# UCL/gp_emulator

Hardware: AMD Instinct MI355X
Metric: test-points/sec for predict(mean+var+grad), N_train=250 D=11 (higher is better)
Workload: dtype f64

## Files before the change

### gp_emulator_amd/csrc/gp_predict_kernel.hpp

```cpp
#pragma once
#include <hip/hip_runtime.h>
#include <stdint.h>
#include <type_traits>
#include <utility>

namespace gpk {

#ifndef GP_WAVES
#define GP_WAVES 8
#endif
#ifndef GP_WAVES_F32
#define GP_WAVES_F32 12
#endif
#ifndef GP_CHUNK
#define GP_CHUNK 64
#endif
#ifndef GP_CHUNK_F32
#define GP_CHUNK_F32 192
#endif
#ifndef GP_ABLATE
#define GP_ABLATE 0
#endif
#ifndef GP_AHEAD
#define GP_AHEAD 4
#endif
#ifndef GP_AHEAD_F32
#define GP_AHEAD_F32 8
#endif
#ifndef GP_RING_PIN
#define GP_RING_PIN 1
#endif
#ifndef GP_MU_DOUBLE
#define GP_MU_DOUBLE 1
#endif
#ifndef GP_ESTRIN
#define GP_ESTRIN 0
#endif
#ifndef GP_EXP_FUSED
#define GP_EXP_FUSED 1
#endif
#ifndef GP_DOTSPLIT
#define GP_DOTSPLIT 1
#endif
#ifndef GP_GROUP_F64
#define GP_GROUP_F64 1
#endif
#ifndef GP_STAMPS
#define GP_STAMPS 0
#endif
constexpr int kTile = 16;
template <typename T, bool kVar = true> struct Geo {
  static constexpr int kWaves = sizeof(T) == 8 ? GP_WAVES : GP_WAVES_F32;
  static constexpr int kThreads = kWaves * 64;
#ifndef GP_WG_PER_CU_SMALL
#define GP_WG_PER_CU_SMALL 0
#endif
  static constexpr int kWGPerCU = kWaves >= 8 ? 1 : (GP_WG_PER_CU_SMALL > 0 ? GP_WG_PER_CU_SMALL : 8 / kWaves);
  static constexpr int kWavesPerSimd = kWaves >= 8 ? kWaves / 4 : kWGPerCU * kWaves / 4;
  static constexpr int kRowsPerWG = kWaves * kTile;
  static constexpr int kChunk = sizeof(T) == 8 ? GP_CHUNK : GP_CHUNK_F32;
};
#ifndef GP_MG_WAVES
#define GP_MG_WAVES 12
#endif
#ifndef GP_MG_WAVES_F32
#define GP_MG_WAVES_F32 16
#endif
#ifndef GP_MG_WG_PER_CU
#define GP_MG_WG_PER_CU 1
#endif
template <typename T> struct Geo<T, false> {
  static constexpr int kWaves = sizeof(T) == 8 ? GP_MG_WAVES : GP_MG_WAVES_F32;
  static constexpr int kThreads = kWaves * 64;
  static constexpr int kWGPerCU = GP_MG_WG_PER_CU;
  static constexpr int kWavesPerSimd = kWGPerCU * kWaves / 4;
  static constexpr int kRowsPerWG = kWaves * kTile;
  static constexpr int kChunk = 1;
};

typedef double f64x4 __attribute__((ext_vector_type(4)));
typedef float f32x4 __attribute__((ext_vector_type(4)));

template <typename F, int... Is>
__device__ __forceinline__ void static_for_impl(F&& f, std::integer_sequence<int, Is...>) {
  (f(std::integral_constant<int, Is>{}), ...);
}
template <int N, typename F>
__device__ __forceinline__ void static_for(F&& f) {
  static_for_impl(f, std::make_integer_sequence<int, N>{});
}

template <typename T> struct Real;
template <> struct Real<double> {
  typedef f64x4 acc_t;
  static constexpr bool kExpand = true;
  static constexpr int kGroup = GP_GROUP_F64;
  __host__ __device__ static constexpr int own_sub(int r, int g) { return 4 * r + g; }
  __device__ static inline acc_t mfma(double a, double b, acc_t c) {
    return __builtin_amdgcn_mfma_f64_16x16x4f64(a, b, c, 0, 0, 0);
  }
  static constexpr double kRoundMagic = 6755399441055744.0;
  __host__ __device__ static inline double exp_(double x) {
#if GP_EXP_FUSED
    const double s = fma(x, 1.4426950408889634, kRoundMagic);
    const double n = s - kRoundMagic;
    const int ni = (int)(unsigned)__builtin_bit_cast(unsigned long long, s);
#else
    x = __builtin_fmax(x, -1000.0);
    const double n = __builtin_rint(x * 1.4426950408889634);
    const int ni = (int)n;
#endif
    double r = fma(n, -6.93147180559945286e-01, x);
    r = fma(n, -2.31904681384629956e-17, r);
#if GP_ESTRIN
    const double r2 = r * r;
    const double p01 = fma(1.00000000000000666e+00, r, 1.0);
    const double p23 = fma(1.66666666665544028e-01, r, 5.00000000000000555e-01);
    const double p45 = fma(8.33333338566834801e-03, r, 4.16666666665732183e-02);
    const double p67 = fma(1.98411702695461072e-04, r, 1.38888889324666632e-03);
    const double p89 = fma(2.76401812311866076e-06, r, 2.48015043709117912e-05);
    const double r4 = r2 * r2;
    const double q0 = fma(r2, p23, p01);
    const double q1 = fma(r2, p67, p45);
    const double q2 = fma(r2, 2.76263485910095559e-07, p89);
    const double r8 = r4 * r4;
    const double s0 = fma(r4, q1, q0);
    const double p = fma(r8, q2, s0);
#else
    double p = 2.76263485910095559e-07;
    p = fma(p, r, 2.76401812311866076e-06);
    p = fma(p, r, 2.48015043709117912e-05);
    p = fma(p, r, 1.98411702695461072e-04);
    p = fma(p, r, 1.38888889324666632e-03);
    p = fma(p, r, 8.33333338566834801e-03);
    p = fma(p, r, 4.16666666665732183e-02);
    p = fma(p, r, 1.66666666665544028e-01);
    p = fma(p, r, 5.00000000000000555e-01);
    p = fma(p, r, 1.00000000000000666e+00);
    p = fma(p, r, 1.0);
#endif
    return ldexp(p, ni);
  }
  __host__ __device__ static inline double exp_clamped(double x) { return exp_(__builtin_fmax(x, -1000.0)); }
  template <int GP>
  __device__ static inline void exp_n(double (&x)[GP]) {
    double n[GP], r[GP], p[GP];
    int ni[GP];
#pragma unroll
    for (int u = 0; u < GP; ++u) x[u] = __builtin_fmax(x[u], -1000.0);
#if GP_EXP_FUSED
#pragma unroll
    for (int u = 0; u < GP; ++u) r[u] = fma(x[u], 1.4426950408889634, kRoundMagic);
#pragma unroll
    for (int u = 0; u < GP; ++u) {
      n[u] = r[u] - kRoundMagic;
      ni[u] = (int)(unsigned)__builtin_bit_cast(unsigned long long, r[u]);
    }
#else
#pragma unroll
    for (int u = 0; u < GP; ++u) {
      n[u] = __builtin_rint(x[u] * 1.4426950408889634);
      ni[u] = (int)n[u];
    }
#endif
#pragma unroll
    for (int u = 0; u < GP; ++u) r[u] = fma(n[u], -6.93147180559945286e-01, x[u]);
#pragma unroll
    for (int u = 0; u < GP; ++u) r[u] = fma(n[u], -2.31904681384629956e-17, r[u]);
#pragma unroll
    for (int u = 0; u < GP; ++u) p[u] = 2.76263485910095559e-07;
    constexpr double c[10] = {2.76401812311866076e-06, 2.48015043709117912e-05, 1.98411702695461072e-04,
                              1.38888889324666632e-03, 8.33333338566834801e-03, 4.16666666665732183e-02,
                              1.66666666665544028e-01, 5.00000000000000555e-01, 1.00000000000000666e+00, 1.0};
#pragma unroll
    for (int j = 0; j < 10; ++j) {
#pragma unroll
      for (int u = 0; u < GP; ++u) p[u] = fma(p[u], r[u], c[j]);
    }
#pragma unroll
    for (int u = 0; u < GP; ++u) x[u] = ldexp(p[u], ni[u]);
  }
  static constexpr double kMaxHalfNorm2 = 67108864.0;
  static constexpr double kFarG = 134217728.0;
};
template <> struct Real<float> {
  typedef f32x4 acc_t;
  static constexpr bool kExpand = false;
#ifndef GP_GROUP_F32
#define GP_GROUP_F32 2
#endif
  static constexpr int kGroup = GP_GROUP_F32;
  __host__ __device__ static constexpr int own_sub(int r, int g) { return 4 * g + r; }
  __device__ static inline acc_t mfma(float a, float b, acc_t c) {
    return __builtin_amdgcn_mfma_f32_16x16x4f32(a, b, c, 0, 0, 0);
  }
  __device__ static inline float exp_(float x) { return __expf(x); }
  __device__ static inline float exp_clamped(float x) { return __expf(x); }
  template <int GP>
  __device__ static inline void exp_n(float (&x)[GP]) {
#pragma unroll
    for (int u = 0; u < GP; ++u) x[u] = __expf(x[u]);
  }
};

template <typename T>
__host__ __device__ constexpr int own_index(int I, int s, int g) {
  return 16 * I + Real<T>::own_sub(s, g);
}

template <typename T>
__host__ __device__ constexpr int point_slot(int n) {
  return 16 * (n / 16) + Real<T>::own_sub((n % 16) / 4, n % 4);
}
template <typename T>
__host__ __device__ constexpr int slot_point(int slot) {
  for (int q = 0; q < 16; ++q)
    if (Real<T>::own_sub(q / 4, q % 4) == slot % 16) return 16 * (slot / 16) + q;
  return -1;
}

struct FragId { int I, J, s; };
__host__ __device__ constexpr int frag_count(int NB) { return NB * (NB + 1) / 2 * 4; }
__host__ __device__ constexpr int frag_col_offset(int J, int NB) { return J * NB - J * (J - 1) / 2; }
__host__ __device__ constexpr FragId frag_at(int n, int NB) {
  const int pair = n >> 2;
  int J = 0;
  while (J + 1 < NB && frag_col_offset(J + 1, NB) <= pair) ++J;
  return FragId{J + pair - frag_col_offset(J, NB), J, n & 3};
}
__host__ __device__ constexpr int frag_index(int I, int J, int s, int NB) {
  return (frag_col_offset(J, NB) + (I - J)) * 4 + s;
}
__host__ __device__ constexpr int frag_count_padded(int NB, int chunk) {
  return (frag_count(NB) + chunk - 1) / chunk * chunk;
}

__host__ __device__ constexpr int row_stride(int D) { return (D + 2 + 3) & ~3; }
#ifndef GP_XA_PAD
#define GP_XA_PAD 1
#endif
template <typename T> __host__ __device__ constexpr int xa_lds_stride(int D) {
  return (GP_XA_PAD && sizeof(T) == 4 && row_stride(D) % 16 == 0) ? row_stride(D) + 4 : row_stride(D);
}

#ifndef GP_FRAG_BUFS
#define GP_FRAG_BUFS 3
#endif
#ifndef GP_FRAG_BUFS_F32
#define GP_FRAG_BUFS_F32 2
#endif
#ifndef GP_SEAM
#define GP_SEAM 2
#endif
constexpr int kLdsBudget = 160 * 1024;
constexpr int kLdsSlack = 32;
template <typename T>
__host__ __device__ constexpr int predict_lds_bytes(int D, int NK, int bufs) {
  const int NP = 16 * ((NK + 3) / 4);
  return (int)sizeof(T) * (NP * xa_lds_stride<T>(D) + bufs * Geo<T>::kChunk * 64 + (2 * D + 1) + 2 * D +
                           2 * Geo<T>::kWaves * kTile * D) + kLdsSlack;
}
template <typename T>
__host__ __device__ constexpr int frag_buffers(int D, int NK) {
  const int want = sizeof(T) == 8 ? GP_FRAG_BUFS : GP_FRAG_BUFS_F32;
  return want > 2 && predict_lds_bytes<T>(D, NK, want) <= kLdsBudget ? want : 2;
}

template <typename T>
struct PredictArgs {
  const T* xa;
  const T* frags;
  const T* sd;
  const T* testing;
  T* mu;
  T* var;
  T* deriv;
  long long M;
  int d_actual;
  int deriv_row_major;
  int n_emulators;
  long long xa_stride, frags_stride, sd_stride;
  unsigned long long* dbg;
  int rows_prescaled;
};

template <int XOR>
__device__ __forceinline__ unsigned swap_halves(unsigned x, unsigned& other) {
  if constexpr (XOR == 16) {
    auto r = __builtin_amdgcn_permlane16_swap(x, x, false, false);
    other = r[1];
    return r[0];
  } else {
    auto r = __builtin_amdgcn_permlane32_swap(x, x, false, false);
    other = r[1];
    return r[0];
  }
}
template <int XOR>
__device__ __forceinline__ float pair_sum(float v) {
  unsigned o, a = swap_halves<XOR>(__float_as_uint(v), o);
  return __uint_as_float(a) + __uint_as_float(o);
}
template <int XOR>
__device__ __forceinline__ double pair_sum(double v) {
  const unsigned long long u = (unsigned long long)__double_as_longlong(v);
  unsigned lo_o, hi_o;
  const unsigned lo_a = swap_halves<XOR>((unsigned)u, lo_o);
  const unsigned hi_a = swap_halves<XOR>((unsigned)(u >> 32), hi_o);
  const double a = __longlong_as_double((long long)(((unsigned long long)hi_a << 32) | lo_a));
  const double o = __longlong_as_double((long long)(((unsigned long long)hi_o << 32) | lo_o));
  return a + o;
}

template <typename T, int N>
__device__ inline void xor_reduce_groups_n(T* v) {
#pragma unroll
  for (int i = 0; i < N; ++i) v[i] = pair_sum<32>(pair_sum<16>(v[i]));
}

template <typename T>
__device__ inline T xor_reduce_groups(T v) {
  return pair_sum<32>(pair_sum<16>(v));
}

template <typename T, int kWaves = Geo<T>::kWaves, int kChunk = Geo<T>::kChunk>
__device__ __forceinline__ void stage_chunk(const T* src, T* dst, int wave, int lane) {
  constexpr int kBytes = kChunk * 64 * (int)sizeof(T);
  constexpr int kPieces = kBytes / 1024;
  static_assert(kPieces * 1024 == kBytes, "chunk must be whole 1 KiB pieces");
  const unsigned voff = (unsigned)lane * 16u;
  const unsigned lds0 = (unsigned)(uintptr_t)(
      (__attribute__((address_space(3))) char*)(reinterpret_cast<char*>(dst)));
#pragma unroll
  for (int pc0 = 0; pc0 < kPieces; pc0 += kWaves) {
    const int pc = pc0 + wave;
    if (pc0 + kWaves <= kPieces || pc < kPieces) {
      const char* s = reinterpret_cast<const char*>(src) + pc * 1024;
      const unsigned m0v = __builtin_amdgcn_readfirstlane(lds0 + pc * 1024);
      unsigned keep;
      asm volatile(
          "s_mov_b32 %0, m0\n\t"
          "s_mov_b32 m0, %1\n\t"
          "s_nop 4\n\t"
          "global_load_lds_dwordx4 %2, %3\n\t"
          "s_mov_b32 m0, %0"
          : "=&s"(keep)
          : "s"(m0v), "v"(voff), "s"(s)
          : "memory");
    }
  }
}
template <typename T, int NP>
__device__ __forceinline__ void stage_pieces(const T* src, T* dst, int first_piece, int lane) {
  const unsigned voff = (unsigned)lane * 16u;
  const unsigned lds0 = (unsigned)(uintptr_t)(
      (__attribute__((address_space(3))) char*)(reinterpret_cast<char*>(dst)));
#pragma unroll
  for (int i = 0; i < NP; ++i) {
    const int pc = first_piece + i;
    const char* s = reinterpret_cast<const char*>(src) + pc * 1024;
    const unsigned m0v = __builtin_amdgcn_readfirstlane(lds0 + pc * 1024);
    unsigned keep;
    asm volatile(
        "s_mov_b32 %0, m0\n\t"
        "s_mov_b32 m0, %1\n\t"
        "s_nop 4\n\t"
        "global_load_lds_dwordx4 %2, %3\n\t"
        "s_mov_b32 m0, %0"
        : "=&s"(keep)
        : "s"(m0v), "v"(voff), "s"(s)
        : "memory");
  }
}
__device__ __forceinline__ void dma_wait() { asm volatile("s_waitcnt vmcnt(0)" ::: "memory"); }

#if GP_STAMPS == 1
#define GP_STAMP(seg)                                                                    \
  do {                                                                                   \
    __builtin_amdgcn_sched_barrier(0);                                                   \
    unsigned long long now_;                                                             \
    asm volatile("s_memtime %0\n\ts_waitcnt lgkmcnt(0)" : "=s"(now_)::"memory");         \
    __builtin_amdgcn_sched_barrier(0);                                                   \
    seg_sum[seg] += now_ - seg_t0;                                                       \
    seg_t0 = now_;                                                                       \
  } while (0)
#else
#define GP_STAMP(seg) do { } while (0)
#endif

template <typename T, int D, int NK, bool kVar = true>
__global__ __launch_bounds__((Geo<T, kVar>::kThreads), (Geo<T, kVar>::kWavesPerSimd)) void predict_kernel(PredictArgs<T> p) {
  typedef Real<T> R;
  typedef Geo<T, kVar> G;
  constexpr int kThreads = G::kThreads;
  constexpr int kRowsPerWG = G::kRowsPerWG;
  typedef typename R::acc_t acc_t;
  constexpr int NB = (NK + 3) / 4;
  constexpr int KL = NK - 4 * (NB - 1);
  constexpr int NP = 16 * NB;
  constexpr int DSG = row_stride(D);
  constexpr int DS = xa_lds_stride<T>(D);
  constexpr int NF = frag_count(NB);
  constexpr int kChunk = G::kChunk;
  constexpr int NCH = (NF + kChunk - 1) / kChunk;
  constexpr int kBufs = kVar ? frag_buffers<T>(D, NK) : 1;
  constexpr int kLook = kBufs - 2;
  constexpr bool kSeamOk = kVar && kBufs == 3 && NCH >= 3 && NCH % 3 == 0;
  constexpr bool kSeamAblated = (GP_ABLATE == 5 || GP_ABLATE == 6) && kSeamOk;
  constexpr bool kSeam = GP_SEAM && !kSeamAblated && kSeamOk;
  constexpr bool kSeamTop = kSeam || kSeamAblated;
  constexpr bool kSeamAlways = kSeam && GP_SEAM == 2;

  __shared__ __attribute__((aligned(16))) T s_xa[NP * DS];
  __shared__ __attribute__((aligned(16))) T s_fr[kBufs][kVar ? kChunk * 64 : 1];
  __shared__ T s_sd[2 * D + 1];
  __shared__ T s_ts[2 * D];
  __shared__ T s_rows[2][G::kWaves][kTile * D];
  static_assert(!kVar || (int)(sizeof(s_xa) + sizeof(s_fr) + sizeof(s_sd) + sizeof(s_ts) + sizeof(s_rows)) + kLdsSlack ==
                             predict_lds_bytes<T>(D, NK, kBufs), "predict_lds_bytes() does not count the kernel's LDS arrays");

  const int tid = threadIdx.x;
  const int lane = tid & 63;
  const int wave = __builtin_amdgcn_readfirstlane(tid >> 6);
  const int ml = lane & 15;
  const int g = lane >> 4;

  const int n_groups = (int)((p.M + kRowsPerWG - 1) / kRowsPerWG);
  int e = 0, cur_e = -1;
  int grp = blockIdx.x;
  while (grp >= n_groups && e < p.n_emulators) { grp -= n_groups; ++e; }

  constexpr int NJ = (kTile * D + 63) / 64;
  auto fetch_rows = [&](int grp_, T (&regs)[NJ]) {
    const long long e0 = ((long long)grp_ * kRowsPerWG + wave * kTile) * p.d_actual;
    const long long emax = p.M * p.d_actual - 1;
#pragma unroll
    for (int j = 0; j < NJ; ++j) {
      long long e_ = e0 + lane + 64 * j;
      e_ = e_ < emax ? e_ : emax;
      regs[j] = p.testing[e_];
    }
  };
  auto stash_rows = [&](int buf_, const T (&regs)[NJ]) {
#pragma unroll
    for (int j = 0; j < NJ; ++j) asm volatile("" ::"v"(regs[j]));
#pragma unroll
    for (int j = 0; j < NJ; ++j)
      if (lane + 64 * j < kTile * p.d_actual) s_rows[buf_][wave][lane + 64 * j] = regs[j];
  };
  int rbuf = 0;
  T rregs[NJ];
  if (e < p.n_emulators) {
    fetch_rows(grp, rregs);
    stash_rows(0, rregs);
  }
#if GP_STAMPS
  unsigned long long seg_sum[8] = {0, 0, 0, 0, 0, 0, 0, 0};
  unsigned long long seg_t0;
  asm volatile("s_memtime %0\n\ts_waitcnt lgkmcnt(0)" : "=s"(seg_t0)::"memory");
#endif

  for (; e < p.n_emulators;) {
    const T* frags = p.frags + e * p.frags_stride;
    auto open_ring = [&]() {
      __syncthreads();
      static_for<1 + kLook>([&](auto cc) {
        constexpr int c = decltype(cc)::value;
        if constexpr (c < NCH) stage_chunk<T, G::kWaves, kChunk>(frags + c * kChunk * 64, &s_fr[c][0], wave, lane);
      });
    };
    if (e != cur_e) {
      cur_e = e;
      if constexpr (kSeamAlways) dma_wait();
      __syncthreads();
      const T* xa = p.xa + e * p.xa_stride;
      for (int i = tid; i < NP * DSG; i += kThreads) s_xa[(i / DSG) * DS + i % DSG] = xa[i];
      const T* sdp = p.sd + e * p.sd_stride;
      if (tid < 2 * D + 1) {
        const bool live = tid == 2 * D || (tid % D) < p.d_actual;
        s_sd[tid] = live ? sdp[tid] : T(0);
        if (tid < 2 * D)
          s_ts[tid] = !live ? T(0) : !p.rows_prescaled ? sdp[tid] : tid < D ? T(1) : T(0);
      }
      if constexpr (!kVar) __syncthreads();
      if constexpr (kVar && kSeamTop) open_ring();
    }
    T* o_mu = p.mu + e * p.M;
    T* o_der = p.deriv + e * p.M * p.d_actual;
    const long long m = (long long)grp * kRowsPerWG + wave * kTile + ml;
    const long long mc = m < p.M ? m : p.M - 1;

    if constexpr (kVar) {
      if constexpr (!kSeamTop) open_ring();
    } else {
      (void)frags;
      __builtin_amdgcn_fence(__ATOMIC_ACQ_REL, "wavefront");
      __builtin_amdgcn_wave_barrier();
    }
    const T b = s_sd[2 * D];
    GP_STAMP(0);

    T t[D];
    T gm = T(0);
    {
      T sdv[D], cv[D], rv[D];
#pragma unroll
      for (int d = 0; d < D; ++d) {
        const int dc = d < p.d_actual ? d : p.d_actual - 1;
        sdv[d] = s_ts[d];
        cv[d] = s_ts[D + d];
        rv[d] = s_rows[rbuf][wave][ml * p.d_actual + dc];
      }
#pragma unroll
      for (int d = 0; d < D; ++d) {
        t[d] = sdv[d] * (rv[d] - cv[d]);
        gm = fma(t[d], t[d], gm);
      }
    }
    gm *= T(-0.5);
    const T poison = gm - gm;
    if constexpr (R::kExpand && GP_EXP_FUSED) {
      const bool in_reach = gm >= T(-R::kFarG);
#pragma unroll
      for (int d = 0; d < D; ++d) t[d] = in_reach ? t[d] : T(0);
      gm = in_reach ? gm : T(-R::kFarG);
    }

    asm volatile("" :: "v"(gm));
    int e_next = e, grp_next = grp + gridDim.x;
    while (grp_next >= n_groups && e_next < p.n_emulators) { grp_next -= n_groups; ++e_next; }
    fetch_rows(e_next < p.n_emulators ? grp_next : grp, rregs);
    const bool ahead = kSeam && e_next == e;

    GP_STAMP(1);
    T kv[NK];
#if GP_MU_DOUBLE
    double mu = 0.0;
#else
    T mu = T(0);
#endif
    T ga[D];
#pragma unroll
    for (int d = 0; d < D; ++d) ga[d] = T(0);

    constexpr int GP = R::kGroup;
    static_for<(NK + GP - 1) / GP>([&](auto qc) {
      constexpr int q0 = decltype(qc)::value * GP;
      constexpr int GU = NK - q0 < GP ? NK - q0 : GP;
      T x[GP][D];
      T al[GP];
      T k[GP];
#pragma unroll
      for (int u = 0; u < GU; ++u) {
        const int q = q0 + u;
        const int i = own_index<T>(q >> 2, q & 3, g);
        const T* row = &s_xa[i * DS];
#pragma unroll
        for (int d = 0; d < D; ++d) x[u][d] = row[d];
        al[u] = row[D];
        if constexpr (R::kExpand) k[u] = row[D + 1] + gm;
      }
#pragma unroll
      for (int u = 0; u < GU; ++u) {
#if GP_ABLATE == 2
        continue;
#endif
        if constexpr (R::kExpand) {
          T part[GP_DOTSPLIT];
          part[0] = k[u];
#pragma unroll
          for (int c = 1; c < GP_DOTSPLIT; ++c) part[c] = T(0);
#pragma unroll
          for (int d = 0; d < D; ++d) part[d % GP_DOTSPLIT] = fma(x[u][d], t[d], part[d % GP_DOTSPLIT]);
#pragma unroll
          for (int c = 1; c < GP_DOTSPLIT; ++c) part[0] += part[c];
          k[u] = part[0];
        } else {
          T r2 = T(0);
#pragma unroll
          for (int d = 0; d < D; ++d) {
            x[u][d] -= t[d];
            r2 = fma(x[u][d], x[u][d], r2);
          }
          k[u] = T(-0.5) * r2;
        }
      }
#pragma unroll
      for (int u = 0; u < GU; ++u) {
#if GP_ABLATE == 2
        k[u] = x[u][0] + t[0];
#else
        k[u] = R::kExpand ? R::exp_(k[u]) : b * R::exp_(k[u]);
#endif
        if constexpr (kVar) kv[q0 + u] = k[u];
      }
#pragma unroll
      for (int u = 0; u < GU; ++u) {
        const T w = k[u] * al[u];
        mu += (decltype(mu))w;
#if GP_ABLATE == 2
        ga[u % D] += w;
#else
#pragma unroll
        for (int d = 0; d < D; ++d) ga[d] = fma(w, x[u][d], ga[d]);
#endif
      }
    });
    GP_STAMP(2);
    const T mu_t = (T)xor_reduce_groups(mu) + poison;
    static_for<(D + 5) / 6>([&](auto bc) {
      constexpr int d0 = decltype(bc)::value * 6;
      constexpr int nb_ = (D - d0 < 6) ? (D - d0) : 6;
      xor_reduce_groups_n<T, nb_>(&ga[d0]);
    });
    {
      T sdv[D];
#pragma unroll
      for (int d = 0; d < D; ++d) sdv[d] = s_sd[d];
#pragma unroll
      for (int d = 0; d < D; ++d)
        ga[d] = R::kExpand ? sdv[d] * fma(-t[d], mu_t, ga[d]) : fma(sdv[d], ga[d], poison);
    }

    if (m < p.M) {
      if (g == 0) o_mu[m] = mu_t;
      int gs = g;
      asm volatile("" : "+v"(gs));
      T gq[(D + 3) / 4];
#pragma unroll
      for (int q = 0; q < (D + 3) / 4; ++q) {
        gq[q] = ga[4 * q];
#pragma unroll
        for (int u = 1; u < 4; ++u)
          if (4 * q + u < D) gq[q] = gs == u ? ga[4 * q + u] : gq[q];
      }
      if (p.deriv_row_major) {
        T* o_row = o_der + m * p.d_actual + gs;
#pragma unroll
        for (int q = 0; q < (D + 3) / 4; ++q)
          if (4 * q + gs < p.d_actual) o_row[4 * q] = gq[q];
      } else {
        T* o_row = o_der + gs * p.M + m;
#pragma unroll
        for (int q = 0; q < (D + 3) / 4; ++q)
          if (4 * q + gs < p.d_actual) o_row[4 * q * p.M] = gq[q];
      }
    }

    GP_STAMP(3);
    stash_rows(rbuf ^ 1, rregs);
    if constexpr (!kVar) {
      rbuf ^= 1;
      e = e_next;
      grp = grp_next;
      continue;
    } else {

    T* o_var = p.var + e * p.M;
    T vacc = T(0);
    acc_t acc;
    constexpr int kAhead = sizeof(T) == 4 ? GP_AHEAD_F32 : GP_AHEAD;
    T afr[kAhead];
#if GP_ABLATE == 1
    static_for<NK>([&](auto qc) { vacc += kv[decltype(qc)::value]; });
    static_for<0>([&](auto fc) {
#else
    static_for<NF>([&](auto fc) {
#endif
      constexpr int f = decltype(fc)::value;
      constexpr int c = f / kChunk, fl = f % kChunk;
      constexpr FragId fid = frag_at(f, NB);
      constexpr int I = fid.I, J = fid.J, s = fid.s;
      if constexpr (fl == 0) {
#if GP_ABLATE == 4
        if constexpr (c == 0) { dma_wait(); __syncthreads(); }
#else
        if constexpr (c == 0 || c + kLook < NCH) {
          dma_wait();
          if constexpr (kLook > 0) {
            if constexpr (c > 0) __builtin_amdgcn_sched_barrier(0);
            asm volatile("s_barrier" ::: "memory");
            if constexpr (c > 0) __builtin_amdgcn_sched_barrier(0);
          } else {
            __syncthreads();
          }
          if constexpr (c + kLook + 1 < NCH) {
            stage_chunk<T, G::kWaves, kChunk>(frags + (c + kLook + 1) * kChunk * 64,
                                              &s_fr[(c + kLook + 1) % kBufs][0], wave, lane);
          } else if constexpr (kSeam && c == NCH - 2) {
            if (kSeamAlways || ahead) stage_chunk<T, G::kWaves, kChunk>(frags, &s_fr[0][0], wave, lane);
          }
        } else if constexpr (GP_ABLATE == 6 && kSeamAblated && c == NCH - 1) {
          __builtin_amdgcn_sched_barrier(0);
          asm volatile("s_barrier" ::: "memory");
          __builtin_amdgcn_sched_barrier(0);
        } else if constexpr (kSeam && c == NCH - 1) {
          if (kSeamAlways || ahead) {
            __builtin_amdgcn_sched_barrier(0);
            asm volatile("s_barrier" ::: "memory");
            __builtin_amdgcn_sched_barrier(0);
            stage_chunk<T, G::kWaves, kChunk>(frags + kChunk * 64, &s_fr[1][0], wave, lane);
          }
        }
#endif
        static_for<kAhead - 1>([&](auto jc) {
          constexpr int n = f + decltype(jc)::value;
          if constexpr (n < NF && (c == 0 || n / kChunk > c - 1 + kLook)) {
#if GP_ABLATE >= 3
            afr[n % kAhead] = kv[n % NK];
#else
            afr[n % kAhead] = s_fr[(n / kChunk) % kBufs][(n % kChunk) * 64 + lane];
#endif
          }
        });
      }
      {
        constexpr int n = f + kAhead - 1;
        if constexpr (n < NF && n / kChunk <= c + kLook) {
#if GP_ABLATE >= 3
          afr[n % kAhead] = kv[(f + 1) % NK];
#else
          afr[n % kAhead] = s_fr[(n / kChunk) % kBufs][(n % kChunk) * 64 + lane];
#endif
        }
      }
      if constexpr (I == J && s == 0) acc = acc_t{T(0), T(0), T(0), T(0)};
      if constexpr (4 * I + s < NK) acc = R::mfma(afr[f % kAhead], kv[4 * I + s], acc);
#if GP_RING_PIN
      if constexpr (sizeof(T) == 4 || GP_RING_PIN > 1) __builtin_amdgcn_sched_barrier(0);
#endif
      if constexpr (I == NB - 1 && s == 3) {
#pragma unroll
        for (int r = 0; r < (J == NB - 1 ? KL : 4); ++r) vacc = fma(acc[r], kv[4 * J + r], vacc);
      }
    });
    rbuf ^= 1;
    GP_STAMP(4);
    vacc = xor_reduce_groups(vacc);
    if (m < p.M && g == 1) o_var[m] = b - vacc + poison;

    e = e_next;
    grp = grp_next;
    GP_STAMP(5);
    }
  }
  if constexpr (kSeamAlways) dma_wait();
#if GP_STAMPS
  if (lane == 0 && p.dbg) {
    for (int k_ = 0; k_ < 8; ++k_) atomicAdd(&p.dbg[k_], seg_sum[k_]);
    atomicAdd(&p.dbg[7], 1ull);
  }
#endif
}

}
```

Measured before the change: 772.3 million.

## Add optional row-prefetch, lagged fold, var-flush deferral and reorder first chunk stage

Adds several compile-time options to the variance pipeline: computing the next tile's row distances mid-loop, folding MFMA accumulators one block late with double-buffered accumulators, and deferring the variance reduction and store to the next iteration. Only the top-order option is on by default. It moves the staging of the (kLook+1)th fragment chunk out of the chunk-0 barrier into the MFMA stream right after the first fragment, so the LDS staging overlaps compute. Row setup is also refactored into a batched lambda. The other options are off by default and add code complexity and register pressure when enabled.

```diff
diff --git a/gp_emulator_amd/csrc/gp_predict_kernel.hpp b/gp_emulator_amd/csrc/gp_predict_kernel.hpp
--- a/gp_emulator_amd/csrc/gp_predict_kernel.hpp
+++ b/gp_emulator_amd/csrc/gp_predict_kernel.hpp
@@ -20,6 +20,33 @@
 #endif
 #ifndef GP_ABLATE
 #define GP_ABLATE 0
+#endif
+#ifndef GP_FOLD_LAG
+#define GP_FOLD_LAG 0
+#endif
+#ifndef GP_FOLD_AT
+#define GP_FOLD_AT 1
+#endif
+#ifndef GP_FOLD_PIN
+#define GP_FOLD_PIN 1
+#endif
+#ifndef GP_TOP_ORDER
+#define GP_TOP_ORDER 1
+#endif
+#ifndef GP_TOP_AT
+#define GP_TOP_AT 0
+#endif
+#ifndef GP_ROWS_EARLY
+#define GP_ROWS_EARLY 0
+#endif
+#ifndef GP_ROWS_BATCH
+#define GP_ROWS_BATCH 4
+#endif
+#ifndef GP_ROWS_AT
+#define GP_ROWS_AT 8
+#endif
+#ifndef GP_VAR_LATE
+#define GP_VAR_LATE 0
 #endif
 #ifndef GP_AHEAD
 #define GP_AHEAD 4
@@ -460,6 +487,19 @@
   asm volatile("s_memtime %0\n\ts_waitcnt lgkmcnt(0)" : "=s"(seg_t0)::"memory");
 #endif
 
+  constexpr bool kRowsEarly = GP_ROWS_EARLY && kVar && GP_ABLATE != 1 && GP_ABLATE != 8;
+  constexpr bool kVarLate = GP_VAR_LATE && kVar && GP_ABLATE != 9;
+  T t[D];
+  T gm = T(0), poison = T(0), poison_nx = T(0);
+  bool rows_ready = false;
+  T pv_vacc = T(0), pv_poison = T(0), pv_b = T(0);
+  long long pv_m = -1;
+  T* pv_var = p.var;
+  auto flush_var = [&]() {
+    const T v = xor_reduce_groups(pv_vacc);
+    if (pv_m >= 0 && g == 1) pv_var[pv_m] = pv_b - v + pv_poison;
+  };
+
   for (; e < p.n_emulators;) {
     const T* frags = p.frags + e * p.frags_stride;
     auto open_ring = [&]() {
@@ -471,6 +511,7 @@
     };
     if (e != cur_e) {
       cur_e = e;
+      rows_ready = false;
       if constexpr (kSeamAlways) dma_wait();
       __syncthreads();
       const T* xa = p.xa + e * p.xa_stride;
@@ -500,39 +541,56 @@
     const T b = s_sd[2 * D];
     GP_STAMP(0);
 
-    T t[D];
-    T gm = T(0);
+    auto row_setup = [&](int buf_, T& gm_, T& poison_, auto batch_c) {
+    constexpr int kB = decltype(batch_c)::value;
+    gm_ = T(0);
+#if GP_ABLATE == 8
+#pragma unroll
+    for (int d = 0; d < D; ++d) t[d] = T(ml + (grp & 3)) * T(0.03125 * (d + 1));
+    gm_ = T(-1);
+#else
     {
-      T sdv[D], cv[D], rv[D];
-#pragma unroll
-      for (int d = 0; d < D; ++d) {
-        const int dc = d < p.d_actual ? d : p.d_actual - 1;
-        sdv[d] = s_ts[d];
-        cv[d] = s_ts[D + d];
-        rv[d] = s_rows[rbuf][wave][ml * p.d_actual + dc];
-      }
-#pragma unroll
-      for (int d = 0; d < D; ++d) {
-        t[d] = sdv[d] * (rv[d] - cv[d]);
-        gm = fma(t[d], t[d], gm);
-      }
-    }
-    gm *= T(-0.5);
-    const T poison = gm - gm;
-    if constexpr (R::kExpand && GP_EXP_FUSED) {
-      const bool in_reach = gm >= T(-R::kFarG);
+      int mlo = ml;
+      if constexpr (kRowsEarly) asm volatile("" : "+v"(mlo));
+      static_for<(D + kB - 1) / kB>([&](auto bc) {
+        constexpr int d0 = decltype(bc)::value * kB;
+        constexpr int nb_ = D - d0 < kB ? D - d0 : kB;
+        T sdv[kB], cv[kB], rv[kB];
+#pragma unroll
+        for (int u = 0; u < nb_; ++u) {
+          const int d = d0 + u;
+          const int dc = d < p.d_actual ? d : p.d_actual - 1;
+          sdv[u] = s_ts[d];
+          cv[u] = s_ts[D + d];
+          rv[u] = s_rows[buf_][wave][mlo * p.d_actual + dc];
+        }
+#pragma unroll
+        for (int u = 0; u < nb_; ++u) {
+          t[d0 + u] = sdv[u] * (rv[u] - cv[u]);
+          gm_ = fma(t[d0 + u], t[d0 + u], gm_);
+        }
+      });
+    }
+#endif
+    gm_ *= T(-0.5);
+    poison_ = gm_ - gm_;
+    if constexpr (R::kExpand && GP_EXP_FUSED && GP_ABLATE != 8) {
+      const bool in_reach = gm_ >= T(-R::kFarG);
 #pragma unroll
       for (int d = 0; d < D; ++d) t[d] = in_reach ? t[d] : T(0);
-      gm = in_reach ? gm : T(-R::kFarG);
-    }
-
-    asm volatile("" :: "v"(gm));
+      gm_ = in_reach ? gm_ : T(-R::kFarG);
+    }
+
+    asm volatile("" :: "v"(gm_));
+    };
+    if (!kRowsEarly || !rows_ready) row_setup(rbuf, gm, poison, std::integral_constant<int, D>{});
     int e_next = e, grp_next = grp + gridDim.x;
     while (grp_next >= n_groups && e_next < p.n_emulators) { grp_next -= n_groups; ++e_next; }
     fetch_rows(e_next < p.n_emulators ? grp_next : grp, rregs);
     const bool ahead = kSeam && e_next == e;
 
     GP_STAMP(1);
+    if constexpr (kVarLate) flush_var();
     T kv[NK];
 #if GP_MU_DOUBLE
     double mu = 0.0;
@@ -658,7 +716,9 @@
 
     T* o_var = p.var + e * p.M;
     T vacc = T(0);
-    acc_t acc;
+    constexpr bool kFoldLag = GP_FOLD_LAG && GP_ABLATE != 1 && GP_ABLATE != 7;
+    constexpr bool kTopOrder = GP_TOP_ORDER && GP_ABLATE != 4 && kLook + 1 < NCH;
+    acc_t acc2[2];
     constexpr int kAhead = sizeof(T) == 4 ? GP_AHEAD_F32 : GP_AHEAD;
     T afr[kAhead];
 #if GP_ABLATE == 1
@@ -684,7 +744,8 @@
           } else {
             __syncthreads();
           }
-          if constexpr (c + kLook + 1 < NCH) {
+          if constexpr (kTopOrder && c == 0) {
+          } else if constexpr (c + kLook + 1 < NCH) {
             stage_chunk<T, G::kWaves, kChunk>(frags + (c + kLook + 1) * kChunk * 64,
                                               &s_fr[(c + kLook + 1) % kBufs][0], wave, lane);
           } else if constexpr (kSeam && c == NCH - 2) {
@@ -724,26 +785,72 @@
 #endif
         }
       }
-      if constexpr (I == J && s == 0) acc = acc_t{T(0), T(0), T(0), T(0)};
-      if constexpr (4 * I + s < NK) acc = R::mfma(afr[f % kAhead], kv[4 * I + s], acc);
+      if constexpr (kRowsEarly && f == (NF > kChunk + GP_ROWS_AT ? kChunk + GP_ROWS_AT : NF / 2)) {
+        __builtin_amdgcn_fence(__ATOMIC_ACQ_REL, "wavefront");
+        __builtin_amdgcn_wave_barrier();
+        row_setup(rbuf ^ 1, gm, poison_nx, std::integral_constant<int, (GP_ROWS_BATCH < D ? GP_ROWS_BATCH : D)>{});
+      }
+      constexpr int a = kFoldLag ? (J & 1) : 0;
+      if constexpr (I == J && s == 0) {
+        if constexpr (kFoldLag && GP_FOLD_PIN && J > 0) __builtin_amdgcn_sched_barrier(0);
+        acc2[a] = acc_t{T(0), T(0), T(0), T(0)};
+      }
+      if constexpr (4 * I + s < NK) acc2[a] = R::mfma(afr[f % kAhead], kv[4 * I + s], acc2[a]);
+      if constexpr (kTopOrder && f == (GP_TOP_AT < kChunk - 1 ? GP_TOP_AT : kChunk - 1)) {
+        __builtin_amdgcn_sched_barrier(0);
+        stage_chunk<T, G::kWaves, kChunk>(frags + (kLook + 1) * kChunk * 64, &s_fr[(kLook + 1) % kBufs][0], wave, lane);
+        __builtin_amdgcn_sched_barrier(0);
+      }
 #if GP_RING_PIN
       if constexpr (sizeof(T) == 4 || GP_RING_PIN > 1) __builtin_amdgcn_sched_barrier(0);
 #endif
-      if constexpr (I == NB - 1 && s == 3) {
-#pragma unroll
-        for (int r = 0; r < (J == NB - 1 ? KL : 4); ++r) vacc = fma(acc[r], kv[4 * J + r], vacc);
+      if constexpr (kFoldLag) {
+        constexpr int at = (J == NB - 1 && GP_FOLD_AT > KL - 1) ? KL - 1 : (GP_FOLD_AT < 3 ? GP_FOLD_AT : 3);
+        if constexpr (J > 0 && I == J && s == at) {
+          if constexpr (GP_FOLD_PIN) __builtin_amdgcn_sched_barrier(0);
+#pragma unroll
+          for (int r = 0; r < 4; ++r) vacc = fma(acc2[a ^ 1][r], kv[4 * (J - 1) + r], vacc);
+          if constexpr (GP_FOLD_PIN) __builtin_amdgcn_sched_barrier(0);
+        }
+      } else if constexpr (GP_ABLATE == 7 && I == NB - 1 && s == 3 && J < NB - 1) {
+        const T c0 = acc2[a][0], c1 = acc2[a][1], c2 = acc2[a][2], c3 = acc2[a][3];
+        asm volatile("" ::"v"(c0), "v"(c1), "v"(c2), "v"(c3));
+      } else if constexpr (I == NB - 1 && s == 3) {
+#pragma unroll
+        for (int r = 0; r < (J == NB - 1 ? KL : 4); ++r) vacc = fma(acc2[a][r], kv[4 * J + r], vacc);
       }
     });
+    if constexpr (kFoldLag) {
+#pragma unroll
+      for (int r = 0; r < KL; ++r) vacc = fma(acc2[(NB - 1) & 1][r], kv[4 * (NB - 1) + r], vacc);
+    }
     rbuf ^= 1;
     GP_STAMP(4);
-    vacc = xor_reduce_groups(vacc);
-    if (m < p.M && g == 1) o_var[m] = b - vacc + poison;
+#if GP_ABLATE == 9
+    asm volatile("" ::"v"(vacc), "v"(o_var));
+#else
+    if constexpr (kVarLate) {
+      pv_vacc = vacc;
+      pv_poison = poison;
+      pv_b = b;
+      pv_var = o_var;
+      pv_m = m < p.M ? m : -1;
+    } else {
+      vacc = xor_reduce_groups(vacc);
+      if (m < p.M && g == 1) o_var[m] = b - vacc + poison;
+    }
+#endif
+    if constexpr (kRowsEarly) {
+      poison = poison_nx;
+      rows_ready = true;
+    }
 
     e = e_next;
     grp = grp_next;
     GP_STAMP(5);
     }
   }
+  if constexpr (kVarLate) flush_var();
   if constexpr (kSeamAlways) dma_wait();
 #if GP_STAMPS
   if (lane == 0 && p.dbg) {
```

New measurement: 774.1 million (median of 6 runs). About the same (+0.2%).
